# mfkiwl/fpga-real-time-fft-analyzer

Measured on AMD Instinct MI355X. Metric: 16K-pt frames/sec (window+IIR+FFT), batch=4096, higher is better.
Workload: dtype f32

## Files before the change

### fpga_real_time_fft_analyzer_amd/csrc/chain_f32.hpp

```cpp
#pragma once
#include <type_traits>
#include "chain_f32_dev.hpp"

namespace {

__device__ __forceinline__ float in_scale_of() { return 1.f; }
__device__ __forceinline__ float in_scale_of(float s) { return s; }

constexpr int kThreads = 256;
constexpr int kLdsComplex = 16 * 272;
constexpr int kScrOff = kLdsComplex * 8;
constexpr int kSideOff = kScrOff + 6 * 16 * 8;
constexpr int kLaneOff = kSideOff + 16;
constexpr int kLdsBytes = kLaneOff + 6 * 16 * 16;
constexpr int kLdsOneRound = 65536;
constexpr int kOneRoundMax = 512;
static_assert(kLdsBytes <= kLdsOneRound, "the exchange images and side slots live inside the one-round image");

__device__ __forceinline__ v2f mv_s(const v2f c0, const v2f c1, const v2f v, const v2f add)
{
    v2f r;
    asm("v_pk_fma_f32 %0, %1, %3, %4 op_sel:[0,0,0] op_sel_hi:[1,0,1]\n\t"
        "v_pk_fma_f32 %0, %2, %3, %0 op_sel:[0,1,0] op_sel_hi:[1,1,1]"
        : "=&v"(r) : "s"(c0), "s"(c1), "v"(v), "v"(add));
    return r;
}
__device__ __forceinline__ v2f mv_v(const v2f c0, const v2f c1, const v2f v, const v2f add)
{
    v2f r;
    asm("v_pk_fma_f32 %0, %1, %3, %4 op_sel:[0,0,0] op_sel_hi:[1,0,1]\n\t"
        "v_pk_fma_f32 %0, %2, %3, %0 op_sel:[0,1,0] op_sel_hi:[1,1,1]"
        : "=&v"(r) : "v"(c0), "v"(c1), "v"(v), "v"(add));
    return r;
}
__device__ __forceinline__ v2f mv0_s(const v2f c0, const v2f c1, const v2f v)
{
    v2f r;
    asm("v_pk_mul_f32 %0, %1, %3 op_sel:[0,0] op_sel_hi:[1,0]\n\t"
        "v_pk_fma_f32 %0, %2, %3, %0 op_sel:[0,1,0] op_sel_hi:[1,1,1]"
        : "=&v"(r) : "s"(c0), "s"(c1), "v"(v));
    return r;
}
__device__ __forceinline__ void mv_acc_s(v2f &z, const v2f c0, const v2f c1, const v2f v)
{
    asm("v_pk_fma_f32 %0, %1, %3, %0 op_sel:[0,0,0] op_sel_hi:[1,0,1]\n\t"
        "v_pk_fma_f32 %0, %2, %3, %0 op_sel:[0,1,0] op_sel_hi:[1,1,1]"
        : "+v"(z) : "s"(c0), "s"(c1), "v"(v));
}

template <int N, typename MatT>
__device__ __forceinline__ void scan_level(v2f &z, const MatT &p)
{
    const v2f u = {row_shr<N>(z.x), row_shr<N>(z.y)};
    mv_acc_s(z, v2f{p[0], p[1]}, v2f{p[2], p[3]}, u);
}

__device__ __forceinline__ float mul_to(float a, float b)
{
    float r;
    asm("v_mul_f32 %0, %1, %2" : "=v"(r) : "v"(a), "v"(b));
    return r;
}

template <bool WINGEN, typename InT>
__device__ __forceinline__ void stage_in_chunks(const InT *__restrict__ xin, const float in_scale,
                                                const float4 *__restrict__ wint, const SaIirLaneTab *__restrict__ lt,
                                                unsigned char *smem, int t, v2f (&d)[32])
{
    const int lane = t & 63, wave = t >> 6;
    float4 pq = make_float4(0.f, 0.f, 0.f, 0.f);
    float g0 = 0.f;
    if constexpr (WINGEN) {
        pq = *reinterpret_cast<const float4 *>(&lt->wgen[t][0]);
        g0 = lt->wg0;
    }
    dma_rows(xin, smem, lane, wave);
    asm volatile("s_waitcnt vmcnt(0)" ::: "memory");
    __builtin_amdgcn_sched_barrier(0);
    const v2f Pw = {pq.x, pq.z}, Qw = {pq.y, pq.w}, G0 = {g0, g0}, sc = {in_scale, in_scale};
    unsigned row[2][12];
    row_open(xin, smem, t, row);
#pragma unroll
    for (int g = 0; g < 4; ++g) {
        int sa[8], sb[8];
        row_step(xin, smem, t, row, 0, g, sa);
        row_step(xin, smem, t, row, 1, g, sb);
#pragma unroll
        for (int u = 0; u < 2; ++u) {
            float4 wa = make_float4(0.f, 0.f, 0.f, 0.f), wb = wa;
            if constexpr (!WINGEN) {
                wa = wint[(2 * g + u) * 256 + t];
                wb = wint[(8 + 2 * g + u) * 256 + t];
            }
            const float fa[4] = {wa.x, wa.y, wa.z, wa.w}, fb[4] = {wb.x, wb.y, wb.z, wb.w};
#pragma unroll
            for (int e4 = 0; e4 < 4; ++e4) {
                const int e = 4 * u + e4, j = 8 * g + e;
                const v2f x = v2f{(float)sa[e], (float)sb[e]} * sc;
                v2f w;
                if constexpr (WINGEN) {
                    const v2f cs = {lt->wcs[j][0], lt->wcs[j][1]};
                    asm("v_pk_fma_f32 %0, %1, %2, %3 op_sel:[0,0,0] op_sel_hi:[1,0,1]\n\t"
                        "v_pk_fma_f32 %0, %4, %2, %0 op_sel:[0,1,0] op_sel_hi:[1,1,1]"
                        : "=&v"(w) : "v"(Pw), "s"(cs), "v"(G0), "v"(Qw));
                } else {
                    w = v2f{fa[e4], fb[e4]};
                }
                d[j] = x * w;
            }
        }
    }
}

template <bool WINGEN>
__device__ __forceinline__ void stage_in_chunks(const float *__restrict__ xin, float, const float4 *__restrict__ wint,
                                                const SaIirLaneTab *__restrict__ lt, unsigned char *smem, int t,
                                                v2f (&d)[32])
{
    const float4 *lds4 = reinterpret_cast<const float4 *>(smem);
    const int lane = t & 63, wave = t >> 6;
    float4 pq = make_float4(0.f, 0.f, 0.f, 0.f);
    float g0 = 0.f;
    if constexpr (WINGEN) {
        pq = *reinterpret_cast<const float4 *>(&lt->wgen[t][0]);
        g0 = lt->wg0;
    }
#pragma unroll
    for (int h = 0; h < 2; ++h) {
        if (h == 1) asm volatile("s_waitcnt lgkmcnt(0)" ::: "memory");
        dma_rows(xin, h, smem, lane, wave);
        asm volatile("s_waitcnt vmcnt(0)" ::: "memory");
        __builtin_amdgcn_sched_barrier(0);
        const int sw = row_swizzle(t);
        const v2f Pw = {pq.x, pq.z}, Qw = {pq.y, pq.w}, G0 = {g0, g0};
#pragma unroll
        for (int g = 0; g < 8; ++g) {
            if (g == 4) __builtin_amdgcn_sched_barrier(0);
            const float4 q = lds4[t * 8 + (g ^ sw)];
            const float qv[4] = {q.x, q.y, q.z, q.w};
            if constexpr (WINGEN) {
#pragma unroll
                for (int e = 0; e < 4; ++e) {
                    const int j = 4 * g + e;
                    if (h == 0) {
                        const v2f cs = {lt->wcs[j][0], lt->wcs[j][1]};
                        v2f w;
                        asm("v_pk_fma_f32 %0, %1, %2, %3 op_sel:[0,0,0] op_sel_hi:[1,0,1]\n\t"
                            "v_pk_fma_f32 %0, %4, %2, %0 op_sel:[0,1,0] op_sel_hi:[1,1,1]"
                            : "=&v"(w) : "v"(Pw), "s"(cs), "v"(G0), "v"(Qw));
                        d[j].x = mul_to(qv[e], w.x);
                        d[j].y = w.y;
                    } else {
                        d[j].y = mul_to(qv[e], d[j].y);
                    }
                }
            } else {
                const float4 w = wint[(8 * h + g) * 256 + t];
                if (h == 0) {
                    d[4 * g + 0].x = mul_to(q.x, w.x);
                    d[4 * g + 1].x = mul_to(q.y, w.y);
                    d[4 * g + 2].x = mul_to(q.z, w.z);
                    d[4 * g + 3].x = mul_to(q.w, w.w);
                } else {
                    d[4 * g + 0].y = mul_to(q.x, w.x);
                    d[4 * g + 1].y = mul_to(q.y, w.y);
                    d[4 * g + 2].y = mul_to(q.z, w.z);
                    d[4 * g + 3].y = mul_to(q.w, w.w);
                }
            }
        }
    }
}

__device__ __forceinline__ void tap_fma8(v2f &nAa, v2f &nBa, v2f &nAb, v2f &nBb, const v2f (&tp)[8], const v2f (&y)[8])
{
#define SA_TAP(ACCA, ACCB, T, Y)                                                               \
    "v_pk_fma_f32 %[" ACCA "], %[" T "], %[" Y "], %[" ACCA "] op_sel:[0,0,0] op_sel_hi:[1,0,1]\n\t" \
    "v_pk_fma_f32 %[" ACCB "], %[" T "], %[" Y "], %[" ACCB "] op_sel:[0,1,0] op_sel_hi:[1,1,1]\n\t"
    asm(SA_TAP("a1", "a2", "t0", "y0") SA_TAP("b1", "b2", "t1", "y1") SA_TAP("a1", "a2", "t2", "y2")
            SA_TAP("b1", "b2", "t3", "y3") SA_TAP("a1", "a2", "t4", "y4") SA_TAP("b1", "b2", "t5", "y5")
                SA_TAP("a1", "a2", "t6", "y6") SA_TAP("b1", "b2", "t7", "y7") ""
        : [a1] "+v"(nAa), [a2] "+v"(nBa), [b1] "+v"(nAb), [b2] "+v"(nBb)
        : [t0] "s"(tp[0]), [t1] "s"(tp[1]), [t2] "s"(tp[2]), [t3] "s"(tp[3]), [t4] "s"(tp[4]), [t5] "s"(tp[5]), [t6] "s"(tp[6]),
          [t7] "s"(tp[7]), [y0] "v"(y[0]), [y1] "v"(y[1]), [y2] "v"(y[2]), [y3] "v"(y[3]), [y4] "v"(y[4]), [y5] "v"(y[5]),
          [y6] "v"(y[6]), [y7] "v"(y[7]));
#undef SA_TAP
}

__device__ __forceinline__ void predict_chunk_ends(const v2f (&tp)[16], const v2f q0, const v2f q1, const v2f (&d)[32],
                                                   v2f &zA, v2f &zB)
{
    v2f nAa = {0.f, 0.f}, nBa = {0.f, 0.f}, nAb = {0.f, 0.f}, nBb = {0.f, 0.f};
#pragma unroll
    for (int hh = 0; hh < 2; ++hh) {
#pragma unroll
        for (int j = 0; j < 16; j += 8) {
            const v2f t8[8] = {tp[j], tp[j + 1], tp[j + 2], tp[j + 3], tp[j + 4], tp[j + 5], tp[j + 6], tp[j + 7]};
            const int o = 16 * hh + j;
            const v2f y8[8] = {d[o], d[o + 1], d[o + 2], d[o + 3], d[o + 4], d[o + 5], d[o + 6], d[o + 7]};
            tap_fma8(nAa, nBa, nAb, nBb, t8, y8);
        }
        if (hh == 0) {
            nAa = mv0_s(q0, q1, nAa + nAb);
            nBa = mv0_s(q0, q1, nBa + nBb);
            nAb = v2f{0.f, 0.f};
            nBb = v2f{0.f, 0.f};
        }
    }
    zA = nAa + nAb;
    zB = nBa + nBb;
}

struct SecConsts {
    v2f pc0, pc1, mb0, mb1;
    float b0, b1, b2, a1, a2, flags_bits;
};
template <typename SecT>
__device__ __forceinline__ SecConsts load_consts(const SecT &k)
{
    return {v2f{k.pc[0], k.pc[1]}, v2f{k.pc[2], k.pc[3]}, v2f{k.mback[0], k.mback[1]}, v2f{k.mback[2], k.mback[3]},
            k.c[0], k.c[1], k.c[2], k.c[3], k.c[4], __builtin_bit_cast(float, k.flags)};
}
__device__ __forceinline__ void pin_consts(const SecConsts &c)
{
    asm volatile("" ::"s"(c.pc0), "s"(c.pc1), "s"(c.mb0), "s"(c.mb1), "s"(c.b1), "s"(c.a1), "s"(c.a2), "s"(c.flags_bits));
}

#ifdef SA_STAMP_IIR
#define SA_STAMP_SEC(i) do { if constexpr (SIDX == 2) SA_STAMP(i); } while (0)
#define SA_STAMP_FFT(i) do {} while (0)
#else
#define SA_STAMP_SEC(i) do {} while (0)
#define SA_STAMP_FFT(i) SA_STAMP(i)
#endif
template <bool PREDICT_NEXT, bool UNIT, int SIDX, typename SecT>
__device__ __forceinline__ void iir_section(v2f (&d)[32], const SecT &k, const SecT &knext, const SecConsts c,
                                            SecConsts &cn, const float4 *lanep_lds, float2 *scr_s, int lane, int wave,
                                            v2f &zA, v2f &zB)
{
    SA_STAMP_SEC(3);
    v2f T = mv_s(c.pc0, c.pc1, zA, zB);
    const int flags = __builtin_bit_cast(int, c.flags_bits);
    if (!(flags & 1)) scan_level<1>(T, k.plev[0]);
    if (!(flags & 2)) scan_level<2>(T, k.plev[1]);
    if (!(flags & 4)) scan_level<4>(T, k.plev[2]);
    if (!(flags & 8)) scan_level<8>(T, k.plev[3]);
    const int row = 4 * wave + (lane >> 4);
    if ((lane & 15) == 15) scr_s[row] = make_float2(T.x, T.y);
    const v2f e = {row_shr<1>(T.x), row_shr<1>(T.y)};
    SA_STAMP_SEC(4);
    lds_barrier();
    SA_STAMP_SEC(5);
    v2f cst;
    if (flags & SA_IIR_SKIP_ROWSCAN) {
        const float2 tt = scr_s[(row - 1) & 15];
        cst = v2f{tt.x, tt.y};
    } else {
        const float2 tt = scr_s[lane & 15];
        v2f r = {tt.x, tt.y};
        scan_level<1>(r, k.prow[0]);
        scan_level<2>(r, k.prow[1]);
        scan_level<4>(r, k.prow[2]);
        scan_level<8>(r, k.prow[3]);
        const int src = (lane & 48) | ((row - 1) & 15);
        cst = v2f{lane_get(r.x, src), lane_get(r.y, src)};
    }
    if (row == 0) cst = v2f{0.f, 0.f};
    const float4 lanep = *lanep_lds;
    const v2f aS = mv_v(v2f{lanep.x, lanep.y}, v2f{lanep.z, lanep.w}, cst, e);
    const v2f bS = mv_s(c.pc0, c.pc1, aS, zA);
    const v2f q1 = {aS.x, bS.x}, q2 = {aS.y, bS.y};
    v2f s1 = c.mb0.x * q1 + c.mb1.x * q2, s2 = c.mb0.y * q1 + c.mb1.y * q2;
    v2f tp[16], h0 = {0.f, 0.f}, h1 = {0.f, 0.f};
    if constexpr (PREDICT_NEXT) {
#pragma unroll
        for (int j = 0; j < 16; ++j) tp[j] = v2f{k.mnext[j][0], k.mnext[j][1]};
        h0 = v2f{k.p16next[0], k.p16next[1]};
        h1 = v2f{k.p16next[2], k.p16next[3]};
    }
    const float b0 = c.b0, b1 = c.b1, b2 = c.b2, na1 = -c.a1, na2 = -c.a2;
    SA_STAMP_SEC(6);
#pragma unroll
    for (int j = 0; j < 32; ++j) {
        const v2f x = d[j];
        v2f y;
        if constexpr (UNIT) {
            y = x + s1;
            s1 = na1 * y + (b1 * x + s2);
            s2 = na2 * y + x;
        } else {
            y = b0 * x + s1;
            s1 = na1 * y + (b1 * x + s2);
            s2 = na2 * y + b2 * x;
        }
        d[j] = y;
    }
    SA_STAMP_SEC(7);
    if constexpr (PREDICT_NEXT) {
        cn = load_consts(knext);
        predict_chunk_ends(tp, h0, h1, d, zA, zB);
        pin_consts(cn);
    }
    SA_STAMP_SEC(8);
}

template <int S, int NSEC, bool UNIT, typename PlanT>
__device__ __forceinline__ void iir_sections(v2f (&d)[32], const PlanT &ka, const SaIirLaneTab *__restrict__ lt,
                                             float2 *scr, int lane, int wave, v2f &zA, v2f &zB, const SecConsts c)
{
    if constexpr (S < NSEC) {
        const float4 *lanep = reinterpret_cast<const float4 *>(reinterpret_cast<const unsigned char *>(scr) + (kLaneOff - kScrOff)) +
                              16 * S + (lane & 15);
        SecConsts cn = c;
        iir_section<(S + 1 < NSEC), UNIT, S>(d, ka.sec[S], ka.sec[S + 1 < NSEC ? S + 1 : S], c, cn, lanep, scr + 16 * S, lane,
                                          wave, zA, zB);
        iir_sections<S + 1, NSEC, UNIT>(d, ka, lt, scr, lane, wave, zA, zB, cn);
    }
}

template <int NSEC, bool UNIT, typename PlanT>
__device__ __forceinline__ void iir_cascade(v2f (&d)[32], const PlanT &ka, const SaIirLaneTab *__restrict__ lt,
                                            float2 *scr, int t)
{
    if (t < 16 * NSEC)
        reinterpret_cast<float4 *>(reinterpret_cast<unsigned char *>(scr) + (kLaneOff - kScrOff))[t] =
            *reinterpret_cast<const float4 *>(&lt->p[t >> 4][t & 15][0]);
    const SecConsts c0 = load_consts(ka.sec[0]);
    v2f tp[16];
#pragma unroll
    for (int j = 0; j < 16; ++j) tp[j] = v2f{ka.m0[j][0], ka.m0[j][1]};
    v2f zA, zB;
    predict_chunk_ends(tp, v2f{ka.p16_0[0], ka.p16_0[1]}, v2f{ka.p16_0[2], ka.p16_0[3]}, d, zA, zB);
    pin_consts(c0);
    iir_sections<0, NSEC, UNIT>(d, ka, lt, scr, t & 63, t >> 6, zA, zB, c0);
}

template <typename Et>
__device__ __forceinline__ void stream_out_segment(const Et *__restrict__ seg, Et *__restrict__ g, int t)
{
    constexpr int n = 16 / (int)sizeof(Et);
    const int h = (int)(((size_t)g / sizeof(Et)) & (size_t)(n - 1));
    constexpr int per_thread = 2048 / n / kThreads;
#pragma unroll
    for (int i = 0; i <= per_thread; ++i) {
        const int u = t + kThreads * i;
        if (i == per_thread && (h == 0 || t != 0)) break;
        const int e0 = n * u - h;
        if (e0 >= 0 && e0 + n <= 2048) {
            float v[4];
            if constexpr (n == 2) {
                const float2 a = reinterpret_cast<const float2 *>(seg)[e0], b = reinterpret_cast<const float2 *>(seg)[e0 + 1];
                v[0] = a.x; v[1] = a.y; v[2] = b.x; v[3] = b.y;
            } else {
#pragma unroll
                for (int j = 0; j < 4; ++j) v[j] = reinterpret_cast<const float *>(seg)[e0 + j];
            }
            store_nt(reinterpret_cast<float *>(g + e0), v[0], v[1], v[2], v[3]);
        } else {
#pragma unroll
            for (int j = 0; j < n; ++j)
                if (e0 + j >= 0 && e0 + j < 2048) {
                    if constexpr (n == 2) {
                        const float2 a = reinterpret_cast<const float2 *>(seg)[e0 + j];
                        store_nt(reinterpret_cast<float2 *>(g + e0 + j), a.x, a.y);
                    } else {
                        store_nt(reinterpret_cast<float *>(g + e0 + j), reinterpret_cast<const float *>(seg)[e0 + j]);
                    }
                }
        }
    }
}

__device__ __forceinline__ int zrow_pos(int within, int row)
{
    const int rest = within & 511;
    return rest + (rest >> 5) + 528 * row;
}
__device__ __forceinline__ int zpos_low(int q) { return zrow_pos(q, q >> 9); }
__device__ __forceinline__ int zpos_partner(int w) { return zrow_pos(w, (4 + (w >> 9)) & 7); }

template <int NSEC, bool UNIT, int OUT, bool WINGEN, bool ONE_ROUND, typename InT, typename PlanT>
__device__ __forceinline__ void chain_frame(const InT *__restrict__ in, const float in_scale, void *__restrict__ out,
                                            const int f, unsigned char *smem,
                                            const float4 *__restrict__ winb, const float4 *__restrict__ twT,
                                            const float4 *__restrict__ twB, const float2 *__restrict__ twC,
                                            const SaIirLaneTab *__restrict__ lanetab, const PlanT &ka,
                                            const int mlo = 0, const int mhi = 0)
{
    cf *ldc = reinterpret_cast<cf *>(smem);
    float2 *scr = reinterpret_cast<float2 *>(smem + kScrOff);
    cf *side = reinterpret_cast<cf *>(smem + kSideOff);

    const int t = threadIdx.x;
    const int lane = t & 63;
    const int wave = t >> 6;
    const int lo = lane & 15;
    const int kq = lane >> 4;
    const InT *xin = in + (size_t)f * kFrameElems<InT>;
    constexpr bool IIR = NSEC > 0;
    cf a[32];
#ifdef SA_STAMPS
    if (threadIdx.x == 0 && g_sa_stamps) g_sa_stamps[(size_t)f * 16 + 13] = __builtin_amdgcn_s_memrealtime();
#endif
    SA_STAMP(0);

    if constexpr (IIR) {
        v2f d[32];
        stage_in_chunks<WINGEN>(xin, in_scale, reinterpret_cast<const float4 *>(lanetab->win_t), lanetab, smem, t, d);
        SA_STAMP(1);
        iir_cascade<NSEC, UNIT>(d, ka, lanetab, scr, t);
        SA_STAMP(2);
#pragma unroll
        for (int h = 0; h < 2; ++h) {
            lds_barrier();
            if ((t >> 7) == h) {
                const unsigned zw = (unsigned)(size_t)(__attribute__((address_space(3))) unsigned char *)(smem) +
                                    8u * 33u * (unsigned)(t & 127);
#pragma unroll
                for (int j = 0; j < 16; ++j) {
                    asm volatile("ds_write2_b32 %0, %1, %2 offset0:%3 offset1:%4" ::"v"(zw), "v"(d[2 * j].x), "v"(d[2 * j + 1].x),
                                 "i"(2 * j), "i"(2 * j + 1) : "memory");
                    asm volatile("ds_write2_b32 %0, %1, %2 offset0:%3 offset1:%4" ::"v"(zw), "v"(d[2 * j].y), "v"(d[2 * j + 1].y),
                                 "i"(2 * (16 + j)), "i"(2 * (16 + j) + 1) : "memory");
                }
            }
            lds_barrier();
#pragma unroll
            for (int m = 0; m < 16; ++m) a[safft::brev(16 * h + m, 5)] = ldc[264 * m + 33 * (t >> 5) + (t & 31)];
        }
    } else if constexpr (!std::is_same_v<InT, float>) {
        static_assert(!ONE_ROUND, "the one-round form is float32 only");
        constexpr int kUnit = 16 / (int)sizeof(InT);
        constexpr int kSlabs = kFrameElems<InT> / (64 * kUnit) / (kThreads / 64);
        static_assert(kSlabs * (kThreads / 64) * 1024 == kFrameElems<InT> * (int)sizeof(InT), "the requests cover the frame exactly");
        __builtin_amdgcn_s_setprio(3);
#pragma unroll
        for (int i = 0; i < kSlabs; ++i) {
            const int n = wave * kSlabs + i;
            const InT *src = xin + n * (64 * kUnit) + lane * kUnit;
            __builtin_amdgcn_global_load_lds((const __attribute__((address_space(1))) void *)src,
                                             (__attribute__((address_space(3))) void *)(smem + n * 1024), 16, 0, SA_DMA_AUX);
        }
        __builtin_amdgcn_s_setprio(0);
        __syncthreads();
#pragma unroll
        for (int pp = 0; pp < 16; ++pp) {
            const float4 w = winb[pp * 256 + t];
            const unsigned u0 = image_dword(xin, smem, t, 2 * pp), u1 = image_dword(xin, smem, t, 2 * pp + 1);
            const cf z0 = point_of(xin, u0) * cf{in_scale, in_scale}, z1 = point_of(xin, u1) * cf{in_scale, in_scale};
            a[safft::brev(2 * pp, 5)] = {z0.x * w.x, z0.y * w.y};
            a[safft::brev(2 * pp + 1, 5)] = {z1.x * w.z, z1.y * w.w};
        }
    } else {
        constexpr int kRounds = ONE_ROUND ? 1 : 2;
        constexpr int kSlabs = 32 / kRounds / 2;
        constexpr int kPairs = 16 / kRounds;
#pragma unroll
        for (int h = 0; h < kRounds; ++h) {
            if (h == 1) __syncthreads();
            __builtin_amdgcn_s_setprio(3);
#pragma unroll
            for (int i = 0; i < kSlabs; ++i) {
                const int n = wave * kSlabs + i;
                const float *src = xin + h * 8192 + n * 256 + lane * 4;
                __builtin_amdgcn_global_load_lds((const __attribute__((address_space(1))) void *)src,
                                                 (__attribute__((address_space(3))) void *)(smem + n * 1024), 16, 0, SA_DMA_AUX);
            }
            __builtin_amdgcn_s_setprio(0);
            __syncthreads();
#pragma unroll
            for (int pp = 0; pp < kPairs; ++pp) {
                const float4 w = winb[(kPairs * h + pp) * 256 + t];
                const cf z0 = ldc[256 * (2 * pp) + t];
                const cf z1 = ldc[256 * (2 * pp + 1) + t];
                a[safft::brev(2 * kPairs * h + 2 * pp, 5)] = {z0.x * w.x, z0.y * w.y};
                a[safft::brev(2 * kPairs * h + 2 * pp + 1, 5)] = {z1.x * w.z, z1.y * w.w};
            }
        }
    }

    SA_STAMP_FFT(3);
    float4 an[5];
#pragma unroll
    for (int i = 0; i < 5; ++i) an[i] = twT[i * 256 + t];
    constexpr bool AN5_EARLY = OUT == SA_OUT_MAG_FULL || OUT == SA_OUT_MARKER;
    float4 an5_early = make_float4(0.f, 0.f, 0.f, 0.f);
    if constexpr (AN5_EARLY) an5_early = twT[5 * 256 + t];
    safft::fft_dit<32>(a);
    {
        const cf wb[8] = {{1.f, 0.f}, {an[0].x, an[0].y}, {an[0].z, an[0].w}, {an[1].x, an[1].y},
                          {an[1].z, an[1].w}, {an[2].x, an[2].y}, {an[2].z, an[2].w}, {an[3].x, an[3].y}};
        const cf wa[4] = {{1.f, 0.f}, {an[3].z, an[3].w}, {an[4].x, an[4].y}, {an[4].z, an[4].w}};
#pragma unroll
        for (int k1 = 1; k1 < 32; ++k1) {
            if ((k1 & 7) != 0) a[k1] = safft::cmul(a[k1], wb[k1 & 7]);
            if ((k1 >> 3) != 0) a[k1] = safft::cmul(a[k1], wa[k1 >> 3]);
        }
    }
    SA_STAMP_FFT(4);
    cf p[2][16];
#pragma unroll
    for (int q = 0; q < 2; ++q) {
        lds_barrier();
#pragma unroll
        for (int r = 0; r < 16; ++r) ldc[r * 272 + t] = a[16 * q + r];
        lds_barrier();
        const int row = 4 * wave + kq;
#pragma unroll
        for (int aa = 0; aa < 16; ++aa) p[q][safft::brev(aa, 4)] = ldc[row * 272 + 16 * aa + lo];
    }
    SA_STAMP_FFT(5);
    safft::fft_dit<16>(p[0]);
    safft::fft_dit<16>(p[1]);
#pragma unroll
    for (int pp = 0; pp < 8; ++pp) {
        const float4 w = twB[pp * 16 + lo];
        if (pp > 0) {
            p[0][2 * pp] = safft::cmul(p[0][2 * pp], {w.x, w.y});
            p[1][2 * pp] = safft::cmul(p[1][2 * pp], {w.x, w.y});
        }
        p[0][2 * pp + 1] = safft::cmul(p[0][2 * pp + 1], {w.z, w.w});
        p[1][2 * pp + 1] = safft::cmul(p[1][2 * pp + 1], {w.z, w.w});
    }
    SA_STAMP_FFT(6);
    {
        const int base = (4 * wave + kq) * 272;
#pragma unroll
        for (int q = 0; q < 2; ++q) {
#pragma unroll
            for (int c = 0; c < 16; ++c) ldc[base + c * 17 + lo] = p[q][c];
            __builtin_amdgcn_fence(__ATOMIC_RELEASE, "wavefront");
            __builtin_amdgcn_wave_barrier();
            __builtin_amdgcn_fence(__ATOMIC_ACQUIRE, "wavefront");
#pragma unroll
            for (int b = 0; b < 16; ++b) p[q][safft::brev(b, 4)] = ldc[base + lo * 17 + b];
            __builtin_amdgcn_fence(__ATOMIC_RELEASE, "wavefront");
            __builtin_amdgcn_wave_barrier();
            __builtin_amdgcn_fence(__ATOMIC_ACQUIRE, "wavefront");
        }
    }
    SA_STAMP_FFT(7);
    safft::fft_dit<16>(p[0]);
    safft::fft_dit<16>(p[1]);
    SA_STAMP_FFT(8);
    int ts = t;
    asm volatile("" : "+v"(ts));
    float4 an5 = an5_early;
    if constexpr (!AN5_EARLY) an5 = twT[5 * 256 + ts];
    const cf wP = {an5.x, an5.y}, wPn = {an5.z, an5.w};
    MarkerAcc mk = {-1.f, SA_NPTS, 0.f};
#pragma unroll
    for (int r = 0; r < 2; ++r) {
        lds_barrier();
#pragma unroll
        for (int q = 0; q < 2; ++q) {
            const int k1 = 16 * q + 4 * wave + kq;
#pragma unroll
            for (int dd = 0; dd < 8; ++dd) {
                const int dsel = (r == 0) ? (dd < 4 ? dd : dd + 8) : dd + 4;
                ldc[k1 + 33 * lo + 528 * dd] = p[q][dsel];
            }
        }
        if (r == 0 && t == 0) {
            side[0] = p[0][12];
            side[1] = p[0][4];
        }
        lds_barrier();
        SA_STAMP(9 + r);
        constexpr bool HALF = OUT == SA_OUT_MAG_HALF || OUT == SA_OUT_SPEC_HALF;
        cf Rs[2][5], Is[2][5];
        float mps[2][5], mqs[2][5];
#pragma unroll
        for (int jj = 0; jj < 2; ++jj) {
            if (HALF && jj == 1) __builtin_amdgcn_sched_barrier(0);
            const int q0 = 4 * (t + 256 * jj);
            const int k0 = q0 + 2048 * r;
            cf w[5];
#pragma unroll
            for (int e = 0; e < 4; ++e) w[e] = cmul_s(wP, twC[(2 * r + jj) * 5 + e]);
            {
                const float2 c0 = twC[(2 * r + jj) * 5], c1 = twC[(2 * r + jj + 1) * 5];
                const cf csel = (t == 255) ? cf{c1.x, c1.y} : cf{c0.x, c0.y};
                w[4] = safft::cmul(wPn, csel);
            }
            const int pa = zpos_low(q0), pb = zpos_low(q0 + 4);
            const int pm0 = zpos_partner(2048 - q0), pm4 = zpos_partner(2044 - q0);
            cf zk[5] = {ldc[pa], ldc[pa + 1], ldc[pa + 2], ldc[pa + 3], ldc[pb]};
            cf zm[5] = {ldc[pm0], ldc[pm4 + 3], ldc[pm4 + 2], ldc[pm4 + 1], ldc[pm4]};
            if (r == 0 && q0 == 2044) {
                zk[4] = side[1];
                zm[4] = side[0];
            }
            if (r == 1 && q0 == 0) zm[0] = side[0];
            cf R[5], I[5];
#pragma unroll
            for (int e = 0; e < 5; ++e) split_eval(zk[e], zm[e], w[e], R[e], I[e]);
            if constexpr (OUT == SA_OUT_MARKER) {
                marker_group(R, I, k0, __builtin_amdgcn_readfirstlane(k0), mlo, mhi, mk);
            } else if constexpr (!HALF) {
                split_store<OUT>(R, I, out, f, k0);
            } else if constexpr (OUT == SA_OUT_SPEC_HALF) {
#pragma unroll
                for (int e = 0; e < 5; ++e) {
                    Rs[jj][e] = R[e];
                    Is[jj][e] = I[e];
                }
            } else {
#pragma unroll
                for (int e = 0; e < 5; ++e) {
                    const cf m2 = safft::pk_fma(I[e], I[e], R[e] * R[e]);
                    mps[jj][e] = fast_sqrt(m2.x);
                    mqs[jj][e] = fast_sqrt(m2.y);
                }
            }
        }
        if constexpr (HALF) {
            lds_barrier();
            if constexpr (OUT == SA_OUT_SPEC_HALF) {
                float4 *s0 = reinterpret_cast<float4 *>(smem), *s1 = reinterpret_cast<float4 *>(smem + 2048 * 8);
                float2 *orow = reinterpret_cast<float2 *>(out) + (size_t)f * (SA_MC + 1);
#pragma unroll
                for (int jj = 0; jj < 2; ++jj) {
                    const int q0 = 4 * (t + 256 * jj);
                    const cf(&R)[5] = Rs[jj];
                    const cf(&I)[5] = Is[jj];
                    s0[q0 / 2] = make_float4(R[0].x, I[0].x, R[1].x, I[1].x);
                    s0[q0 / 2 + 1] = make_float4(R[2].x, I[2].x, R[3].x, I[3].x);
                    s1[(2044 - q0) / 2] = make_float4(R[4].y, -I[4].y, R[3].y, -I[3].y);
                    s1[(2044 - q0) / 2 + 1] = make_float4(R[2].y, -I[2].y, R[1].y, -I[1].y);
                    if (r == 0 && q0 == 0) store_nt(orow + SA_MC, R[0].y, -I[0].y);
                }
                lds_barrier();
                stream_out_segment(reinterpret_cast<const float2 *>(smem), orow + 2048 * r, t);
                stream_out_segment(reinterpret_cast<const float2 *>(smem + 2048 * 8), orow + 6144 - 2048 * r, t);
            } else {
                float4 *s0 = reinterpret_cast<float4 *>(smem), *s1 = reinterpret_cast<float4 *>(smem + 2048 * 4);
                float *orow = reinterpret_cast<float *>(out) + (size_t)f * (SA_MC + 1);
#pragma unroll
                for (int jj = 0; jj < 2; ++jj) {
                    const int q0 = 4 * (t + 256 * jj);
                    const float(&mp)[5] = mps[jj];
                    const float(&mq)[5] = mqs[jj];
                    s0[q0 / 4] = make_float4(mp[0], mp[1], mp[2], mp[3]);
                    s1[(2044 - q0) / 4] = make_float4(mq[4], mq[3], mq[2], mq[1]);
                    if (r == 0 && q0 == 0) store_nt(orow + SA_MC, mq[0]);
                }
                lds_barrier();
                stream_out_segment(reinterpret_cast<const float *>(smem), orow + 2048 * r, t);
                stream_out_segment(reinterpret_cast<const float *>(smem + 2048 * 4), orow + 6144 - 2048 * r, t);
            }
        }
    }
    if constexpr (OUT == SA_OUT_MARKER) marker_finish(mk, reinterpret_cast<float4 *>(scr), out, f, t);
    SA_STAMP(11);
#ifdef SA_STAMPS
    __builtin_amdgcn_s_waitcnt(0);
#endif
    SA_STAMP(12);
#ifdef SA_STAMPS
    if (threadIdx.x == 0 && g_sa_stamps) {
        g_sa_stamps[(size_t)f * 16 + 14] = __builtin_amdgcn_s_memrealtime();
        g_sa_stamps[(size_t)f * 16 + 15] =
            (unsigned long long)__builtin_amdgcn_s_getreg((4 << 0) | (0 << 6) | (31 << 11)) |
            ((unsigned long long)__builtin_amdgcn_s_getreg((20 << 0) | (0 << 6) | (31 << 11)) << 32);
    }
#endif
}

template <typename InT, int NSEC, bool UNIT, int OUT, bool WINGEN, bool ONE_ROUND, typename... Scale>
__global__ __launch_bounds__(kThreads, 4) void chain_f32_kernel(const InT *__restrict__ in, const Scale... in_scale,
                                                                 void *__restrict__ out, int batch,
                                                                 const float4 *__restrict__ winb,
                                                                 const float4 *__restrict__ twT,
                                                                 const float4 *__restrict__ twB,
                                                                 const float2 *__restrict__ twC,
                                                                 const SaIirLaneTab *__restrict__ lanetab,
                                                                 const SaIirK ka)
{
    extern __shared__ __attribute__((aligned(16))) unsigned char smem[];
    int f = blockIdx.x;
    if (f >= batch) return;
    chain_frame<NSEC, UNIT, OUT, WINGEN, ONE_ROUND>(in, in_scale_of(in_scale...), out, f, smem, winb, twT, twB, twC,
                                                     lanetab, ka);
// ... 126 lines not shown
```

### fpga_real_time_fft_analyzer_amd/csrc/chain_f32_dev.hpp

```cpp
#pragma once
#include "sa_common.hpp"
#include "fft_regs.hpp"
#include "p12_dev.hpp"
#include "../../include/specan.h"

using safft::cf;
typedef float v2f __attribute__((ext_vector_type(2)));

namespace {

#ifndef SA_DMA_AUX
#define SA_DMA_AUX 2
#endif

__device__ __forceinline__ float fast_sqrt(float v) { return __builtin_amdgcn_sqrtf(v); }

#ifdef SA_STAMPS
__device__ unsigned long long *g_sa_stamps = nullptr;
#define SA_STAMP(i)                                                                        \
    do {                                                                                   \
        __builtin_amdgcn_sched_barrier(0);                                                 \
        if (threadIdx.x == 0 && g_sa_stamps) {     \
            unsigned long long c_;                                                         \
            asm volatile("s_memtime %0\n\ts_waitcnt lgkmcnt(0)" : "=s"(c_)::"memory");     \
            g_sa_stamps[(size_t)blockIdx.x * 16 + (i)] = c_;                               \
        }                                                                                  \
        __builtin_amdgcn_sched_barrier(0);                                                 \
    } while (0)
#else
#define SA_STAMP(i) do {} while (0)
#endif

__device__ __forceinline__ void lds_barrier()
{
    asm volatile("s_waitcnt lgkmcnt(0)\n\ts_barrier" ::: "memory");
}

template <int N>
__device__ __forceinline__ float row_shr(float v)
{
    return __builtin_bit_cast(float, __builtin_amdgcn_update_dpp(0, __builtin_bit_cast(int, v), 0x110 + N, 0xF, 0xF, true));
}

__device__ __forceinline__ float lane_get(float v, int src_lane)
{
    return __builtin_bit_cast(float, __builtin_amdgcn_ds_bpermute(src_lane << 2, __builtin_bit_cast(int, v)));
}

typedef float f4nt __attribute__((ext_vector_type(4)));
typedef float f2nt __attribute__((ext_vector_type(2)));
__device__ __forceinline__ void store_nt(float *p, float a, float b, float c, float d)
{
    __builtin_nontemporal_store(f4nt{a, b, c, d}, reinterpret_cast<f4nt *>(p));
}
__device__ __forceinline__ void store_nt(float2 *p, float a, float b)
{
    __builtin_nontemporal_store(f2nt{a, b}, reinterpret_cast<f2nt *>(p));
}
__device__ __forceinline__ void store_nt(float *p, float a) { __builtin_nontemporal_store(a, p); }

__device__ __forceinline__ int row_swizzle(int r) { return (r >> 1) & 7; }

template <typename T>
__device__ __forceinline__ void dma_rows_impl(const T *x, int h, unsigned char *smem, int lane, int wave)
{
    const int rl = lane >> 3;
    __builtin_amdgcn_s_setprio(3);
#pragma unroll
    for (int i = 0; i < 8; ++i) {
        const int n = wave * 8 + i;
        const int r = 8 * n + rl;
        const int lc = (lane & 7) ^ row_swizzle(r);
        const T *src = x + r * 64 + h * 32 + lc * (16 / (int)sizeof(T));
        __builtin_amdgcn_global_load_lds((const __attribute__((address_space(1))) void *)src,
                                         (__attribute__((address_space(3))) void *)(smem + n * 1024), 16, 0, SA_DMA_AUX);
    }
    __builtin_amdgcn_s_setprio(0);
}
__device__ __forceinline__ void dma_rows(const float *x, int h, unsigned char *smem, int lane, int wave)
{
    dma_rows_impl(x, h, smem, lane, wave);
}
__device__ __forceinline__ void dma_rows(const int16_t *x, unsigned char *smem, int lane, int wave)
{
    dma_rows_impl(x, 0, smem, lane, wave);
}

template <typename InT> constexpr int kFrameElems = SA_NPTS;
template <> constexpr int kFrameElems<SaP12> = SA_P12_FRAME_BYTES;

__device__ __forceinline__ int p12_row_swizzle(int r) { return (r >> 3) & 1; }

__device__ __forceinline__ void dma_rows(const SaP12 *x, unsigned char *smem, int lane, int wave)
{
    __builtin_amdgcn_s_setprio(3);
#pragma unroll
    for (int i = 0; i < 6; ++i) {
        const int n = wave * 6 + i;
        const int s = 64 * n + lane;
        const int u = s ^ p12_row_swizzle(s / 6);
        __builtin_amdgcn_global_load_lds((const __attribute__((address_space(1))) void *)(x + 16 * u),
                                         (__attribute__((address_space(3))) void *)(smem + n * 1024), 16, 0, SA_DMA_AUX);
    }
    __builtin_amdgcn_s_setprio(0);
}

typedef unsigned u4v __attribute__((ext_vector_type(4)));
__device__ __forceinline__ void p12_read_row(const unsigned char *smem, int t, unsigned (&ua)[12], unsigned (&ub)[12])
{
    const unsigned sw = (unsigned)p12_row_swizzle(t);
    const unsigned row = (unsigned)(size_t)(const __attribute__((address_space(3))) unsigned char *)(smem) + 96u * (unsigned)t;
    const unsigned ae = row + 16u * sw, ao = row + 16u * (sw ^ 1u);
    u4v q[6];
    asm volatile("ds_read_b128 %0, %6\n\t"
                 "ds_read_b128 %1, %7\n\t"
                 "ds_read_b128 %2, %6 offset:32\n\t"
                 "ds_read_b128 %3, %7 offset:32\n\t"
                 "ds_read_b128 %4, %6 offset:64\n\t"
                 "ds_read_b128 %5, %7 offset:64\n\t"
                 "s_waitcnt lgkmcnt(0)"
                 : "=&v"(q[0]), "=&v"(q[1]), "=&v"(q[2]), "=&v"(q[3]), "=&v"(q[4]), "=&v"(q[5])
                 : "v"(ae), "v"(ao)
                 : "memory");
#pragma unroll
    for (int c = 0; c < 3; ++c) {
        ua[4 * c] = q[c].x; ua[4 * c + 1] = q[c].y; ua[4 * c + 2] = q[c].z; ua[4 * c + 3] = q[c].w;
        ub[4 * c] = q[3 + c].x; ub[4 * c + 1] = q[3 + c].y; ub[4 * c + 2] = q[3 + c].z; ub[4 * c + 3] = q[3 + c].w;
    }
}

__device__ __forceinline__ void row_open(const int16_t *, const unsigned char *, int, unsigned (&)[2][12]) {}
__device__ __forceinline__ void row_step(const int16_t *, const unsigned char *smem, int t, unsigned (&)[2][12], int h, int g,
                                         int (&s)[8])
{
    const uint4 q = reinterpret_cast<const uint4 *>(smem)[t * 8 + ((g + 4 * h) ^ row_swizzle(t))];
    const unsigned u[4] = {q.x, q.y, q.z, q.w};
#pragma unroll
    for (int e = 0; e < 8; ++e) s[e] = (e & 1) ? (int)u[e >> 1] >> 16 : (int)(short)(u[e >> 1] & 0xFFFFu);
}
__device__ __forceinline__ void row_open(const SaP12 *, const unsigned char *smem, int t, unsigned (&u)[2][12])
{
    p12_read_row(smem, t, u[0], u[1]);
}
__device__ __forceinline__ void row_step(const SaP12 *, const unsigned char *, int, unsigned (&u)[2][12], int h, int g,
                                         int (&s)[8])
{
    p12_unpack8(u[h][3 * g], u[h][3 * g + 1], u[h][3 * g + 2], s);
}

__device__ __forceinline__ unsigned image_dword(const int16_t *, const unsigned char *smem, int t, int m1)
{
    return reinterpret_cast<const unsigned *>(smem)[256 * m1 + t];
}
__device__ __forceinline__ cf point_of(const int16_t *, unsigned u)
{
    return cf{(float)(int)(short)(u & 0xFFFFu), (float)((int)u >> 16)};
}
__device__ __forceinline__ unsigned image_dword(const SaP12 *, const unsigned char *smem, int t, int m1)
{
    const unsigned *ldu = reinterpret_cast<const unsigned *>(smem) + ((3 * t) >> 2);
    const unsigned sh = 8u * ((3u * (unsigned)t) & 3u);
    return __builtin_amdgcn_alignbit(ldu[192 * m1 + 1], ldu[192 * m1], sh);
}
__device__ __forceinline__ cf point_of(const SaP12 *, unsigned u) { return cf{(float)p12_bfe(u, 0), (float)p12_bfe(u, 12)}; }

__device__ __forceinline__ void store_rows(float *o, int h, const unsigned char *smem, int t)
{
    const float4 *lds4 = reinterpret_cast<const float4 *>(smem);
    const int lane = t & 63, wave = t >> 6, rl = lane >> 3;
#pragma unroll
    for (int i = 0; i < 8; ++i) {
        const int n = wave * 8 + i;
        const int r = 8 * n + rl;
        const int lc = (lane & 7) ^ row_swizzle(r);
        const float4 v = lds4[n * 64 + lane];
        store_nt(o + r * 64 + h * 32 + lc * 4, v.x, v.y, v.z, v.w);
    }
}

__device__ __forceinline__ cf cmul_s(const cf a, const float2 wu)
{
    const cf w = {wu.x, wu.y};
    cf t, r;
    asm("v_pk_mul_f32 %0, %2, %3 op_sel:[0,0] op_sel_hi:[0,1]\n\t"
        "v_pk_fma_f32 %1, %2, %3, %0 op_sel:[1,1,0] op_sel_hi:[1,0,1] neg_lo:[0,1,0]"
        : "=&v"(t), "=v"(r) : "v"(a), "s"(w));
    return r;
}

__device__ __forceinline__ void split_eval(const cf zk, const cf zm, const cf w, cf &R, cf &I)
{
    const cf s = zk + zm;
    const cf d = zk - zm;
    cf u, tw;
    asm("v_pk_mul_f32 %0, %4, %6 op_sel:[1,0] op_sel_hi:[1,1]\n\t"
        "v_pk_fma_f32 %1, %5, %6, %0 op_sel:[0,1,0] op_sel_hi:[0,0,1] neg_hi:[0,1,0]\n\t"
        "v_pk_add_f32 %2, %4, %1 op_sel:[0,0] op_sel_hi:[0,0] neg_hi:[0,1]\n\t"
        "v_pk_add_f32 %3, %5, %1 op_sel:[1,1] op_sel_hi:[1,1] neg_hi:[0,1]"
        : "=&v"(u), "=&v"(tw), "=&v"(R), "=v"(I) : "v"(s), "v"(d), "v"(w));
}

template <int OUT>
__device__ __forceinline__ void split_store(const cf (&R)[5], const cf (&I)[5], void *__restrict__ out, int f, int k0)
{
    if constexpr (OUT == SA_OUT_MAG_FULL || OUT == SA_OUT_MAG_HALF) {
        float mp[5], mq[5];
#pragma unroll
        for (int e = 0; e < 5; ++e) {
            const cf m2 = safft::pk_fma(I[e], I[e], R[e] * R[e]);
            mp[e] = fast_sqrt(m2.x);
            mq[e] = fast_sqrt(m2.y);
        }
        if constexpr (OUT == SA_OUT_MAG_FULL) {
            float *o = reinterpret_cast<float *>(out) + (size_t)f * SA_NPTS;
            store_nt(o + k0, mp[0], mp[1], mp[2], mp[3]);
            store_nt(o + SA_NPTS - k0 - 4, mp[4], mp[3], mp[2], mp[1]);
            store_nt(o + SA_MC + k0, mq[0], mq[1], mq[2], mq[3]);
            store_nt(o + SA_MC - k0 - 4, mq[4], mq[3], mq[2], mq[1]);
        } else {
            float *o = reinterpret_cast<float *>(out) + (size_t)f * (SA_MC + 1);
#pragma unroll
            for (int e = 0; e < 4; ++e) store_nt(o + k0 + e, mp[e]);
#pragma unroll
            for (int e = 1; e < 5; ++e) store_nt(o + SA_MC - k0 - e, mq[e]);
            if (k0 == 0) store_nt(o + SA_MC, mq[0]);
        }
    } else {
        float2 *o = reinterpret_cast<float2 *>(out) + (size_t)f * (SA_MC + 1);
#pragma unroll
        for (int e = 0; e < 4; ++e) store_nt(o + k0 + e, R[e].x, I[e].x);
#pragma unroll
        for (int e = 1; e < 5; ++e) store_nt(o + SA_MC - k0 - e, R[e].y, -I[e].y);
        if (k0 == 0) store_nt(o + SA_MC, R[0].y, -I[0].y);
    }
}

struct MarkerAcc {
    float mag;
    int bin;
    float pow;
};

template <bool MASK>
__device__ __forceinline__ void marker_run(MarkerAcc &a, const float (&m)[4], const float (&p)[4], int s, int lo, int hi)
{
    float best = -1.f, pw = 0.f;
    int be = 0;
#pragma unroll
    for (int e = 0; e < 4; ++e) {
        float mm = m[e], pe = p[e];
        if constexpr (MASK) {
            const bool in = (unsigned)(s + e - lo) < (unsigned)(hi - lo);
            mm = in ? mm : -1.f;
            pe = in ? pe : 0.f;
        }
        pw += pe;
        if (mm > best) {
            best = mm;
            be = e;
        }
    }
    a.pow += pw;
    if (best > a.mag || (best == a.mag && s + be < a.bin)) {
        a.mag = best;
        a.bin = s + be;
    }
}

__device__ __forceinline__ void marker_run_any(MarkerAcc &a, const float (&m)[4], const float (&p)[4], int s, int w, int lo,
                                               int hi)
{
    if (w + 256 <= lo || w >= hi) return;
    if (w >= lo && w + 256 <= hi)
        marker_run<false>(a, m, p, s, lo, hi);
    else
        marker_run<true>(a, m, p, s, lo, hi);
}

__device__ __forceinline__ void marker_group(const cf (&R)[5], const cf (&I)[5], int k0, int kw, int lo, int hi, MarkerAcc &a)
{
    float mp[5], mq[5], pp[5], pq[5];
#pragma unroll
    for (int e = 0; e < 5; ++e) {
        const cf m2 = safft::pk_fma(I[e], I[e], R[e] * R[e]);
        pp[e] = m2.x;
        pq[e] = m2.y;
        mp[e] = fast_sqrt(m2.x);
        mq[e] = fast_sqrt(m2.y);
    }
    const float m0[4] = {mp[0], mp[1], mp[2], mp[3]}, p0[4] = {pp[0], pp[1], pp[2], pp[3]};
    const float m1[4] = {mp[4], mp[3], mp[2], mp[1]}, p1[4] = {pp[4], pp[3], pp[2], pp[1]};
    const float m2[4] = {mq[0], mq[1], mq[2], mq[3]}, p2[4] = {pq[0], pq[1], pq[2], pq[3]};
    const float m3[4] = {mq[4], mq[3], mq[2], mq[1]}, p3[4] = {pq[4], pq[3], pq[2], pq[1]};
    marker_run_any(a, m0, p0, k0, kw, lo, hi);
    marker_run_any(a, m1, p1, SA_NPTS - k0 - 4, SA_NPTS - kw - 256, lo, hi);
    marker_run_any(a, m2, p2, SA_MC + k0, SA_MC + kw, lo, hi);
    marker_run_any(a, m3, p3, SA_MC - k0 - 4, SA_MC - kw - 256, lo, hi);
}

__device__ __forceinline__ void marker_merge(MarkerAcc &a, const MarkerAcc &b)
{
// ... 38 lines not shown
```

Measured before the change: 32.84 million.

## Use SGPR-base plus VGPR-offset addressing, stage twB in LDS, seed tap chains with mul

Global addresses are rewritten as a wave-uniform scalar base plus a 32-bit per-lane byte offset, so the compiler can use saddr+voffset addressing instead of full 64-bit per-lane address arithmetic. The twB twiddle table is loaded early and parked in LDS, and the FFT reads it from there instead of from global memory. The tap FMA chains now start with multiplies instead of zero-initialised accumulators, removing a few instructions. LDS grows by the twiddle buffer, and a static assert checks that four workgroups still fit per CU.

```diff
diff --git a/fpga_real_time_fft_analyzer_amd/csrc/chain_f32.hpp b/fpga_real_time_fft_analyzer_amd/csrc/chain_f32.hpp
--- a/fpga_real_time_fft_analyzer_amd/csrc/chain_f32.hpp
+++ b/fpga_real_time_fft_analyzer_amd/csrc/chain_f32.hpp
@@ -12,10 +12,14 @@
 constexpr int kScrOff = kLdsComplex * 8;
 constexpr int kSideOff = kScrOff + 6 * 16 * 8;
 constexpr int kLaneOff = kSideOff + 16;
-constexpr int kLdsBytes = kLaneOff + 6 * 16 * 16;
-constexpr int kLdsOneRound = 65536;
+constexpr int kTwbOff = kLaneOff + 6 * 16 * 16;
+constexpr int kTwbBytes = 8 * 16 * 16;
+constexpr int kLdsBytes = kTwbOff + kTwbBytes;
+constexpr int kOneRoundImage = 65536;
+constexpr int kLdsOneRound = kOneRoundImage + kTwbBytes;
 constexpr int kOneRoundMax = 512;
-static_assert(kLdsBytes <= kLdsOneRound, "the exchange images and side slots live inside the one-round image");
+static_assert(kTwbOff <= kOneRoundImage, "the exchange images and side slots live inside the one-round image");
+static_assert(4 * kLdsBytes <= 160 * 1024, "four workgroups share a CU's LDS");
 
 __device__ __forceinline__ v2f mv_s(const v2f c0, const v2f c1, const v2f v, const v2f add)
 {
@@ -89,8 +93,8 @@
         for (int u = 0; u < 2; ++u) {
             float4 wa = make_float4(0.f, 0.f, 0.f, 0.f), wb = wa;
             if constexpr (!WINGEN) {
-                wa = wint[(2 * g + u) * 256 + t];
-                wb = wint[(8 + 2 * g + u) * 256 + t];
+                wa = *at_bytes(wint + (2 * g + u) * 256, 16u * (unsigned)t);
+                wb = *at_bytes(wint + (8 + 2 * g + u) * 256, 16u * (unsigned)t);
             }
             const float fa[4] = {wa.x, wa.y, wa.z, wa.w}, fb[4] = {wb.x, wb.y, wb.z, wb.w};
 #pragma unroll
@@ -155,7 +159,7 @@
                     }
                 }
             } else {
-                const float4 w = wint[(8 * h + g) * 256 + t];
+                const float4 w = *at_bytes(wint + (8 * h + g) * 256, 16u * (unsigned)t);
                 if (h == 0) {
                     d[4 * g + 0].x = mul_to(q.x, w.x);
                     d[4 * g + 1].x = mul_to(q.y, w.y);
@@ -172,41 +176,63 @@
     }
 }
 
+template <bool FIRST_A, bool FIRST_B>
 __device__ __forceinline__ void tap_fma8(v2f &nAa, v2f &nBa, v2f &nAb, v2f &nBb, const v2f (&tp)[8], const v2f (&y)[8])
 {
 #define SA_TAP(ACCA, ACCB, T, Y)                                                               \
     "v_pk_fma_f32 %[" ACCA "], %[" T "], %[" Y "], %[" ACCA "] op_sel:[0,0,0] op_sel_hi:[1,0,1]\n\t" \
     "v_pk_fma_f32 %[" ACCB "], %[" T "], %[" Y "], %[" ACCB "] op_sel:[0,1,0] op_sel_hi:[1,1,1]\n\t"
-    asm(SA_TAP("a1", "a2", "t0", "y0") SA_TAP("b1", "b2", "t1", "y1") SA_TAP("a1", "a2", "t2", "y2")
-            SA_TAP("b1", "b2", "t3", "y3") SA_TAP("a1", "a2", "t4", "y4") SA_TAP("b1", "b2", "t5", "y5")
-                SA_TAP("a1", "a2", "t6", "y6") SA_TAP("b1", "b2", "t7", "y7") ""
-        : [a1] "+v"(nAa), [a2] "+v"(nBa), [b1] "+v"(nAb), [b2] "+v"(nBb)
-        : [t0] "s"(tp[0]), [t1] "s"(tp[1]), [t2] "s"(tp[2]), [t3] "s"(tp[3]), [t4] "s"(tp[4]), [t5] "s"(tp[5]), [t6] "s"(tp[6]),
-          [t7] "s"(tp[7]), [y0] "v"(y[0]), [y1] "v"(y[1]), [y2] "v"(y[2]), [y3] "v"(y[3]), [y4] "v"(y[4]), [y5] "v"(y[5]),
-          [y6] "v"(y[6]), [y7] "v"(y[7]));
+#define SA_TAP_MUL(ACCA, ACCB, T, Y)                                       \
+    "v_pk_mul_f32 %[" ACCA "], %[" T "], %[" Y "] op_sel:[0,0] op_sel_hi:[1,0]\n\t" \
+    "v_pk_mul_f32 %[" ACCB "], %[" T "], %[" Y "] op_sel:[0,1] op_sel_hi:[1,1]\n\t"
+#define SA_TAPS_2_7                                                                                        \
+    SA_TAP("a1", "a2", "t2", "y2") SA_TAP("b1", "b2", "t3", "y3") SA_TAP("a1", "a2", "t4", "y4")           \
+        SA_TAP("b1", "b2", "t5", "y5") SA_TAP("a1", "a2", "t6", "y6") SA_TAP("b1", "b2", "t7", "y7") ""
+#define SA_TAP_INS                                                                                                          \
+    [t0] "s"(tp[0]), [t1] "s"(tp[1]), [t2] "s"(tp[2]), [t3] "s"(tp[3]), [t4] "s"(tp[4]), [t5] "s"(tp[5]), [t6] "s"(tp[6]),  \
+        [t7] "s"(tp[7]), [y0] "v"(y[0]), [y1] "v"(y[1]), [y2] "v"(y[2]), [y3] "v"(y[3]), [y4] "v"(y[4]), [y5] "v"(y[5]),    \
+        [y6] "v"(y[6]), [y7] "v"(y[7])
+    if constexpr (FIRST_A && FIRST_B)
+        asm(SA_TAP_MUL("a1", "a2", "t0", "y0") SA_TAP_MUL("b1", "b2", "t1", "y1") SA_TAPS_2_7
+            : [a1] "=&v"(nAa), [a2] "=&v"(nBa), [b1] "=&v"(nAb), [b2] "=&v"(nBb)
+            : SA_TAP_INS);
+    else if constexpr (FIRST_B)
+        asm(SA_TAP("a1", "a2", "t0", "y0") SA_TAP_MUL("b1", "b2", "t1", "y1") SA_TAPS_2_7
+            : [a1] "+v"(nAa), [a2] "+v"(nBa), [b1] "=&v"(nAb), [b2] "=&v"(nBb)
+            : SA_TAP_INS);
+    else {
+        static_assert(!FIRST_A, "the (nAa, nBa) chains never start alone");
+        asm(SA_TAP("a1", "a2", "t0", "y0") SA_TAP("b1", "b2", "t1", "y1") SA_TAPS_2_7
+            : [a1] "+v"(nAa), [a2] "+v"(nBa), [b1] "+v"(nAb), [b2] "+v"(nBb)
+            : SA_TAP_INS);
+    }
+#undef SA_TAP_INS
+#undef SA_TAPS_2_7
+#undef SA_TAP_MUL
 #undef SA_TAP
 }
 
 __device__ __forceinline__ void predict_chunk_ends(const v2f (&tp)[16], const v2f q0, const v2f q1, const v2f (&d)[32],
                                                    v2f &zA, v2f &zB)
 {
-    v2f nAa = {0.f, 0.f}, nBa = {0.f, 0.f}, nAb = {0.f, 0.f}, nBb = {0.f, 0.f};
-#pragma unroll
-    for (int hh = 0; hh < 2; ++hh) {
-#pragma unroll
-        for (int j = 0; j < 16; j += 8) {
-            const v2f t8[8] = {tp[j], tp[j + 1], tp[j + 2], tp[j + 3], tp[j + 4], tp[j + 5], tp[j + 6], tp[j + 7]};
-            const int o = 16 * hh + j;
-            const v2f y8[8] = {d[o], d[o + 1], d[o + 2], d[o + 3], d[o + 4], d[o + 5], d[o + 6], d[o + 7]};
-            tap_fma8(nAa, nBa, nAb, nBb, t8, y8);
-        }
-        if (hh == 0) {
-            nAa = mv0_s(q0, q1, nAa + nAb);
-            nBa = mv0_s(q0, q1, nBa + nBb);
-            nAb = v2f{0.f, 0.f};
-            nBb = v2f{0.f, 0.f};
-        }
-    }
+    v2f nAa, nBa, nAb, nBb;
+    const auto y8_at = [&](int o, v2f (&y8)[8]) {
+#pragma unroll
+        for (int i = 0; i < 8; ++i) y8[i] = d[o + i];
+    };
+    const v2f tlo[8] = {tp[0], tp[1], tp[2], tp[3], tp[4], tp[5], tp[6], tp[7]};
+    const v2f thi[8] = {tp[8], tp[9], tp[10], tp[11], tp[12], tp[13], tp[14], tp[15]};
+    v2f y8[8];
+    y8_at(0, y8);
+    tap_fma8<true, true>(nAa, nBa, nAb, nBb, tlo, y8);
+    y8_at(8, y8);
+    tap_fma8<false, false>(nAa, nBa, nAb, nBb, thi, y8);
+    nAa = mv0_s(q0, q1, nAa + nAb);
+    nBa = mv0_s(q0, q1, nBa + nBb);
+    y8_at(16, y8);
+    tap_fma8<false, true>(nAa, nBa, nAb, nBb, tlo, y8);
+    y8_at(24, y8);
+    tap_fma8<false, false>(nAa, nBa, nAb, nBb, thi, y8);
     zA = nAa + nAb;
     zB = nBa + nBb;
 }
@@ -324,7 +350,7 @@
 {
     if (t < 16 * NSEC)
         reinterpret_cast<float4 *>(reinterpret_cast<unsigned char *>(scr) + (kLaneOff - kScrOff))[t] =
-            *reinterpret_cast<const float4 *>(&lt->p[t >> 4][t & 15][0]);
+            *at_bytes(reinterpret_cast<const float4 *>(&lt->p[0][0][0]), 16u * (unsigned)t);
     const SecConsts c0 = load_consts(ka.sec[0]);
     v2f tp[16];
 #pragma unroll
@@ -403,10 +429,17 @@
     if (threadIdx.x == 0 && g_sa_stamps) g_sa_stamps[(size_t)f * 16 + 13] = __builtin_amdgcn_s_memrealtime();
 #endif
     SA_STAMP(0);
+    float4 *twb_lds = reinterpret_cast<float4 *>(smem + (ONE_ROUND ? kOneRoundImage : kTwbOff));
+    float4 twb_mine = make_float4(0.f, 0.f, 0.f, 0.f);
+    if (t < kTwbBytes / 16) twb_mine = twB[t];
+    const auto park_twb = [&] {
+        if (t < kTwbBytes / 16) twb_lds[t] = twb_mine;
+    };
 
     if constexpr (IIR) {
         v2f d[32];
         stage_in_chunks<WINGEN>(xin, in_scale, reinterpret_cast<const float4 *>(lanetab->win_t), lanetab, smem, t, d);
+        park_twb();
         SA_STAMP(1);
         iir_cascade<NSEC, UNIT>(d, ka, lanetab, scr, t);
         SA_STAMP(2);
@@ -437,11 +470,12 @@
 #pragma unroll
         for (int i = 0; i < kSlabs; ++i) {
             const int n = wave * kSlabs + i;
-            const InT *src = xin + n * (64 * kUnit) + lane * kUnit;
+            const InT *src = at_bytes(xin + (uniform_wave(wave) * kSlabs + i) * (64 * kUnit), 16u * (unsigned)lane);
             __builtin_amdgcn_global_load_lds((const __attribute__((address_space(1))) void *)src,
                                              (__attribute__((address_space(3))) void *)(smem + n * 1024), 16, 0, SA_DMA_AUX);
         }
         __builtin_amdgcn_s_setprio(0);
+        park_twb();
         __syncthreads();
 #pragma unroll
         for (int pp = 0; pp < 16; ++pp) {
@@ -462,11 +496,12 @@
 #pragma unroll
             for (int i = 0; i < kSlabs; ++i) {
                 const int n = wave * kSlabs + i;
-                const float *src = xin + h * 8192 + n * 256 + lane * 4;
+                const float *src = at_bytes(xin + h * 8192 + (uniform_wave(wave) * kSlabs + i) * 256, 16u * (unsigned)lane);
                 __builtin_amdgcn_global_load_lds((const __attribute__((address_space(1))) void *)src,
                                                  (__attribute__((address_space(3))) void *)(smem + n * 1024), 16, 0, SA_DMA_AUX);
             }
             __builtin_amdgcn_s_setprio(0);
+            if (h == 0) park_twb();
             __syncthreads();
 #pragma unroll
             for (int pp = 0; pp < kPairs; ++pp) {
@@ -482,10 +517,10 @@
     SA_STAMP_FFT(3);
     float4 an[5];
 #pragma unroll
-    for (int i = 0; i < 5; ++i) an[i] = twT[i * 256 + t];
+    for (int i = 0; i < 5; ++i) an[i] = *at_bytes(twT + i * 256, 16u * (unsigned)t);
     constexpr bool AN5_EARLY = OUT == SA_OUT_MAG_FULL || OUT == SA_OUT_MARKER;
     float4 an5_early = make_float4(0.f, 0.f, 0.f, 0.f);
-    if constexpr (AN5_EARLY) an5_early = twT[5 * 256 + t];
+    if constexpr (AN5_EARLY) an5_early = *at_bytes(twT + 5 * 256, 16u * (unsigned)t);
     safft::fft_dit<32>(a);
     {
         const cf wb[8] = {{1.f, 0.f}, {an[0].x, an[0].y}, {an[0].z, an[0].w}, {an[1].x, an[1].y},
@@ -514,7 +549,7 @@
     safft::fft_dit<16>(p[1]);
 #pragma unroll
     for (int pp = 0; pp < 8; ++pp) {
-        const float4 w = twB[pp * 16 + lo];
+        const float4 w = twb_lds[pp * 16 + lo];
         if (pp > 0) {
             p[0][2 * pp] = safft::cmul(p[0][2 * pp], {w.x, w.y});
             p[1][2 * pp] = safft::cmul(p[1][2 * pp], {w.x, w.y});
@@ -546,7 +581,7 @@
     int ts = t;
     asm volatile("" : "+v"(ts));
     float4 an5 = an5_early;
-    if constexpr (!AN5_EARLY) an5 = twT[5 * 256 + ts];
+    if constexpr (!AN5_EARLY) an5 = *at_bytes(twT + 5 * 256, 16u * (unsigned)ts);
     const cf wP = {an5.x, an5.y}, wPn = {an5.z, an5.w};
     MarkerAcc mk = {-1.f, SA_NPTS, 0.f};
 #pragma unroll
@@ -598,7 +633,7 @@
             if constexpr (OUT == SA_OUT_MARKER) {
                 marker_group(R, I, k0, __builtin_amdgcn_readfirstlane(k0), mlo, mhi, mk);
             } else if constexpr (!HALF) {
-                split_store<OUT>(R, I, out, f, k0);
+                split_store<OUT>(R, I, out, f, k0, t);
             } else if constexpr (OUT == SA_OUT_SPEC_HALF) {
 #pragma unroll
                 for (int e = 0; e < 5; ++e) {
diff --git a/fpga_real_time_fft_analyzer_amd/csrc/chain_f32_dev.hpp b/fpga_real_time_fft_analyzer_amd/csrc/chain_f32_dev.hpp
--- a/fpga_real_time_fft_analyzer_amd/csrc/chain_f32_dev.hpp
+++ b/fpga_real_time_fft_analyzer_amd/csrc/chain_f32_dev.hpp
@@ -1,4 +1,5 @@
 #pragma once
+#include <type_traits>
 #include "sa_common.hpp"
 #include "fft_regs.hpp"
 #include "p12_dev.hpp"
@@ -36,6 +37,17 @@
     asm volatile("s_waitcnt lgkmcnt(0)\n\ts_barrier" ::: "memory");
 }
 
+template <typename T>
+__device__ __forceinline__ T *at_bytes(T *base, unsigned lane_bytes)
+{
+    using Byte = std::conditional_t<std::is_const_v<T>, const unsigned char, unsigned char>;
+    asm("" : "+s"(base));
+    asm("" : "+v"(lane_bytes));
+    using GlobalByte = __attribute__((address_space(1))) Byte;
+    return reinterpret_cast<T *>((Byte *)((GlobalByte *)reinterpret_cast<Byte *>(base) + lane_bytes));
+}
+__device__ __forceinline__ int uniform_wave(int wave) { return __builtin_amdgcn_readfirstlane(wave); }
+
 template <int N>
 __device__ __forceinline__ float row_shr(float v)
 {
@@ -64,14 +76,15 @@
 template <typename T>
 __device__ __forceinline__ void dma_rows_impl(const T *x, int h, unsigned char *smem, int lane, int wave)
 {
+    constexpr int kRow = 64 * (int)sizeof(T);
     const int rl = lane >> 3;
+    const unsigned v0 = (unsigned)(rl * kRow + (((lane & 7) ^ (rl >> 1)) << 4)), v1 = v0 ^ 64u;
+    const T *xw = x + uniform_wave(wave) * (64 * 64) + h * 32;
     __builtin_amdgcn_s_setprio(3);
 #pragma unroll
     for (int i = 0; i < 8; ++i) {
         const int n = wave * 8 + i;
-        const int r = 8 * n + rl;
-        const int lc = (lane & 7) ^ row_swizzle(r);
-        const T *src = x + r * 64 + h * 32 + lc * (16 / (int)sizeof(T));
+        const T *src = at_bytes(xw + i * (8 * 64), (i & 1) ? v1 : v0);
         __builtin_amdgcn_global_load_lds((const __attribute__((address_space(1))) void *)src,
                                          (__attribute__((address_space(3))) void *)(smem + n * 1024), 16, 0, SA_DMA_AUX);
     }
@@ -93,13 +106,14 @@
 
 __device__ __forceinline__ void dma_rows(const SaP12 *x, unsigned char *smem, int lane, int wave)
 {
+    const int uw = uniform_wave(wave);
     __builtin_amdgcn_s_setprio(3);
 #pragma unroll
     for (int i = 0; i < 6; ++i) {
         const int n = wave * 6 + i;
         const int s = 64 * n + lane;
-        const int u = s ^ p12_row_swizzle(s / 6);
-        __builtin_amdgcn_global_load_lds((const __attribute__((address_space(1))) void *)(x + 16 * u),
+        const unsigned v = (unsigned)((lane ^ p12_row_swizzle(s / 6)) << 4);
+        __builtin_amdgcn_global_load_lds((const __attribute__((address_space(1))) void *)at_bytes(x + 1024 * (uw * 6 + i), v),
                                          (__attribute__((address_space(3))) void *)(smem + n * 1024), 16, 0, SA_DMA_AUX);
     }
     __builtin_amdgcn_s_setprio(0);
@@ -201,7 +215,7 @@
 }
 
 template <int OUT>
-__device__ __forceinline__ void split_store(const cf (&R)[5], const cf (&I)[5], void *__restrict__ out, int f, int k0)
+__device__ __forceinline__ void split_store(const cf (&R)[5], const cf (&I)[5], void *__restrict__ out, int f, int k0, int t)
 {
     if constexpr (OUT == SA_OUT_MAG_FULL || OUT == SA_OUT_MAG_HALF) {
         float mp[5], mq[5];
@@ -213,10 +227,12 @@
         }
         if constexpr (OUT == SA_OUT_MAG_FULL) {
             float *o = reinterpret_cast<float *>(out) + (size_t)f * SA_NPTS;
-            store_nt(o + k0, mp[0], mp[1], mp[2], mp[3]);
-            store_nt(o + SA_NPTS - k0 - 4, mp[4], mp[3], mp[2], mp[1]);
-            store_nt(o + SA_MC + k0, mq[0], mq[1], mq[2], mq[3]);
-            store_nt(o + SA_MC - k0 - 4, mq[4], mq[3], mq[2], mq[1]);
+            const unsigned up = 16u * (unsigned)t, dn = 16u * (unsigned)(SA_NTHREADS - 1 - t);
+            const int kc = k0 - 4 * t;
+            store_nt(at_bytes(o + kc, up), mp[0], mp[1], mp[2], mp[3]);
+            store_nt(at_bytes(o + (SA_NPTS - 4 * SA_NTHREADS - kc), dn), mp[4], mp[3], mp[2], mp[1]);
+            store_nt(at_bytes(o + (SA_MC + kc), up), mq[0], mq[1], mq[2], mq[3]);
+            store_nt(at_bytes(o + (SA_MC - 4 * SA_NTHREADS - kc), dn), mq[4], mq[3], mq[2], mq[1]);
         } else {
             float *o = reinterpret_cast<float *>(out) + (size_t)f * (SA_MC + 1);
 #pragma unroll
```

After: 33.37 million, median of 6. 1.02x the previous value.
